# kevinh-e/BetaOne

Measured on AMD Instinct MI355X. Metric: mcts_nodes_per_sec, higher is better.
Workload: dtype f32 (3 x f16 split, f32 accumulate)

## Files before the change

betaone_amd/csrc/bo_engine.cpp:

```cpp
#include "../../include/betaone_engine.h"
#include "../../include/betaone_lab.h"

#include "bo_tree.h"
#include "bo_fastw.h"
#include "bo_info.h"
#include "bo_select_wide.h"
#include "bo_replay.h"
#include "bo_train.h"
#include "bo_metrics.h"
#include "bo_pgn.h"
#include "bo_san.h"
#include "bo_analyse.h"
#include "bo_reanalyse.h"
#include "bo_perft.h"
#include "bo_mate.h"
#include "bo_anchor.h"
#include "bo_book.h"
#include "bo_merge.h"
#include "bo_tb.h"
#include "bo_nn_fused.h"
#include "bo_conv.h"
#include "bo_tower.h"
#include "bo_tower_wg.h"
#include "bo_tower_h.h"
// ... 202 lines not shown
    e->fast = fast;
    double per_sim = 1.0;
    for (int k = 1; k <= cfg->mcts_batch_size; k++) {
        const double r = (double)(int)(cfg->widen_coeff * sqrt((double)k)) / (double)k;
        if (r > per_sim) per_sim = r;
    }
    c.NCAP = fast ? 2 : (int)ceil(c.S * per_sim) + 2 * root_m + 4;
    c.nstride = c.NCAP;
    c.PLY_CAP = cfg->max_plies; c.TRK_CAP = cfg->max_plies;
    c.UL_MAX = fast ? 1 : c.B; c.CH_MAX = ch_max < 1 ? 1 : ch_max;
    c.cpuct = (float)cfg->cpuct;
    c.keep = (float)(1.0 - cfg->dirichlet_epsilon);
    c.eps = cfg->dirichlet_epsilon;
    c.use_noise = cfg->dirichlet_alpha > 0 ? 1 : 0;
    c.root_m = root_m;
    c.profile = 0;
    { const char *v = getenv("BETAONE_BURST_TWO_PATHS"); c.burst_two = (v && v[0] == '0') ? 0 : 1; }
    c.root_q = 0;
    const size_t G = (size_t)c.G, N = G * (size_t)c.NCAP;
    Eng &d = e->d;
    int rc = 0;
    float *sq = nullptr, *rcp = nullptr; int *wl = nullptr;
    rc |= e->alloc(&sq, (size_t)c.S + 2); rc |= e->alloc(&wl, (size_t)c.B + 1); rc |= e->alloc(&rcp, (size_t)c.S + 3);
    int **iscal[] = {&d.sims_done, &d.n_nodes, &d.rows, &d.n_runs, &d.n_ul, &d.req_nlegal, &d.status,
                     &d.trk_n, &d.n_hist, &d.ctx_mode, &d.root_nch, &d.stat_evals,
                     &d.stat_flushes, &d.stat_term_sims, &d.stat_levels, &d.stat_children_scanned, &e->d_go, &e->d_action};
    for (int **p : iscal) rc |= e->alloc(p, G);
    const size_t res_ints = G * (4 + 2 * (size_t)BO_RES_CAP) + 4, info_ints = G * 18;
    rc |= e->alloc(&e->d_res_blk, res_ints); rc |= e->alloc(&e->d_info_blk, info_ints);
    if (!rc) {
        d.res_n = e->d_res_blk; d.res_best_idx = e->d_res_blk + G; d.res_best_mv = e->d_res_blk + 2 * G; d.res_total = e->d_res_blk + 3 * G;
        d.res_idx = e->d_res_blk + 4 * G; d.res_val = reinterpret_cast<float *>(e->d_res_blk + 4 * G + G * BO_RES_CAP);
        d.res_watch = e->d_res_blk + G * (4 + 2 * (size_t)BO_RES_CAP); d.watch = nullptr; d.watch_n = 1;
        d.phase = e->d_info_blk; d.req_node = e->d_info_blk + G; d.root_nlegal = e->d_info_blk + 2 * G; d.root_term = e->d_info_blk + 3 * G;
        d.ply = e->d_info_blk + 4 * G;
        e->d_turn_action = e->d_info_blk + 5 * G; e->d_turn_state = e->d_info_blk + 6 * G; e->d_turn_cres = e->d_info_blk + 7 * G;
        e->d_turn_rv = reinterpret_cast<float *>(e->d_info_blk + 15 * G); e->d_turn_resigned = e->d_info_blk + 16 * G;
        e->d_turn_rnext = e->d_info_blk + 17 * G;
        rt_memset(e->d_res_blk, 0, res_ints * 4, nullptr); rt_memset(e->d_info_blk, 0, info_ints * 4, nullptr);
    }
    rc |= rt_host_alloc((void **)&e->h_res, res_ints * 4); rc |= rt_host_alloc((void **)&e->h_info, info_ints * 4);
    rc |= rt_host_alloc((void **)&e->h_noise, G * BO_MAX_MOVES * sizeof(double)); rc |= rt_host_alloc((void **)&e->h_go, G * 4);
    rc |= rt_host_alloc((void **)&e->h_action, 2 * G * 4);
    rc |= rt_host_alloc((void **)&e->h_turn_u, G * sizeof(double)); rc |= rt_host_alloc((void **)&e->h_turn_flags, G * 4);
    rc |= e->alloc(&e->d_turn_pw, (size_t)cfg->num_simulations + 1);
    { const char *v = getenv("BETAONE_TURN_COPIES"); e->ship = !(v && v[0] == '1'); }
// ... 35 lines not shown
        rc |= e->alloc(&st, (size_t)BO_FW_SQRT_TAB); rc |= e->alloc(&rt, (size_t)BO_FW_RCP_TAB);
        if (!rc) {
            std::vector<float> hs2(BO_FW_SQRT_TAB), hr2(BO_FW_RCP_TAB, 0.0f);
            for (int n = 0; n < BO_FW_SQRT_TAB; n++) hs2[n] = (float)sqrt((double)n);
            for (int k = 1; k < BO_FW_RCP_TAB; k++) hr2[k] = (float)(1.0 / (double)k);
            rt_h2d(st, hs2.data(), hs2.size() * sizeof(float), nullptr); rt_h2d(rt, hr2.data(), hr2.size() * sizeof(float), nullptr);
            rt_sync(nullptr);
            f.sqrt_tab = st; f.rcp_tab = rt;
            rt_memset(f.ctl, 0, G * (size_t)f.CS * 4, nullptr);
            rt_memset(f.played_now, 0, G * 4, nullptr);
            rt_memset(f.row_val, 0, G * L * 4, nullptr);
            d.played_now = f.played_now;
        }
    }
    if (rc) { bo_engine_destroy(e); return fail(BO_E_HIP, "device allocation failed"); }
    std::vector<float> hs((size_t)c.S + 2);
    for (int n = 0; n < c.S + 2; n++) hs[n] = (float)sqrt((double)n + 1e-8);
    std::vector<int> hw((size_t)c.B + 1);
    for (int k = 0; k <= c.B; k++) hw[k] = (int)(cfg->widen_coeff * sqrt((double)k));
    std::vector<float> hr((size_t)c.S + 3, 0.0f);
    for (int n = 1; n < c.S + 3; n++) hr[n] = (float)(1.0 / (double)n);
    rt_h2d(rcp, hr.data(), hr.size() * sizeof(float), nullptr);
    d.rcp_lut = rcp;
    rt_h2d(sq, hs.data(), hs.size() * sizeof(float), nullptr);
    rt_h2d(wl, hw.data(), hw.size() * sizeof(int), nullptr);
    d.sqrt_lut = sq; d.widen_lut = wl;
    for (int **p : iscal) rt_memset(*p, 0, G * sizeof(int), nullptr);
    rt_memset(d.noise, 0, G * BO_MAX_MOVES * sizeof(double), nullptr);
    rt_sync(nullptr);
    e->h_i32.resize(G);
    e->rng.resize(G);
    for (size_t g = 0; g < G; g++) hr_seed(&e->rng[g], (uint32_t)g);
    memset(e->h_noise, 0, G * BO_MAX_MOVES * sizeof(double));
    e->h_nl.resize(G); e->h_term.resize(G);
    *out = e;
    return BO_OK;
}

extern "C" void bo_engine_destroy(bo_engine *e) {
    if (!e) return;
    rt_set_device(e->device);
    for (void *p : e->allocs) rt_free(p);
    rt_host_free(e->h_res); rt_host_free(e->h_info); rt_host_free(e->h_noise); rt_host_free(e->h_go); rt_host_free(e->h_action);
    rt_host_free(e->h_turn_u); rt_host_free(e->h_turn_flags);
    if (e->ev_turn_made) rt_event_destroy(e->ev_turn);
    for (int i = 0; i < 2; i++) if (e->ev_action_made[i]) rt_event_destroy(e->ev_action[i]);
// ... 191 lines not shown
static int step_launch(bo_engine *e, const float *policy_dev, const float *value_dev, int policy_kind, float *nn_in_dev, void *stream, const StepTail &vt) {
    e->prefetch_valid = false;
    if (e->fast) {
        const int rows = e->d.c.G * e->f.L;
        if (policy_kind != BO_POLICY_NONE) RT(RT_LAUNCH(bo_k_fw_apply, rows, stream, e->d, e->f, policy_dev, value_dev, policy_kind));
#if !defined(BO_WAVE_EMU)
        if (e->sel_profile) {
            if (!e->sel_ev0) { RT((int)hipEventCreate(&e->sel_ev0)); RT((int)hipEventCreate(&e->sel_ev1)); }
            if (e->sel_pending) {
                float ms = 0.0f;
                RT((int)hipEventSynchronize(e->sel_ev1));
                RT((int)hipEventElapsedTime(&ms, e->sel_ev0, e->sel_ev1));
                e->sel_ms += ms; e->sel_launches++; e->sel_pending = 0;
            }
            RT((int)hipEventRecord(e->sel_ev0, (hipStream_t)stream));
        }
#endif
        RT(launch_fw_select(e, policy_kind != BO_POLICY_NONE ? e->f.row_val : value_dev, policy_kind, stream));
#if !defined(BO_WAVE_EMU)
        if (e->sel_profile) { RT((int)hipEventRecord(e->sel_ev1, (hipStream_t)stream)); e->sel_pending = 1; }
#endif
        RT(RT_LAUNCH(bo_k_fw_leaf, rows, stream, e->d, e->f, nn_in_dev));
    } else {
        if (e->d.tb_n > 0 && (e->d.tb_flags & TBF_SEARCH)) RT(RT_LAUNCH(bo_k_step_tb, e->d.c.G, stream, e->d, policy_dev, value_dev, policy_kind, nn_in_dev, vt));
        else RT(RT_LAUNCH(bo_k_step, e->d.c.G, stream, e->d, policy_dev, value_dev, policy_kind, nn_in_dev, vt));
    }
    return BO_OK;
}
extern "C" int bo_step(bo_engine *e, const float *policy_dev, const float *value_dev, int policy_kind, float *nn_in_dev,
                       void *stream) {
    if (!e || !nn_in_dev) return fail(BO_E_ARG, "null argument");
    if (policy_kind != BO_POLICY_NONE && (!policy_dev || !value_dev)) return fail(BO_E_ARG, "policy/value required");
    return step_launch(e, policy_dev, value_dev, policy_kind, nn_in_dev, stream, StepTail{nullptr, nullptr, nullptr, nullptr, 0});
}
extern "C" int bo_step_heads(bo_engine *e, const float *logits_dev, const float *vpart_dev, const float *b1_dev, const float *w2_dev,
                             const float *b2_dev, int rows, float *nn_in_dev, void *stream) {
    if (!e || !nn_in_dev || !logits_dev || !vpart_dev || !b1_dev || !w2_dev || !b2_dev) return fail(BO_E_ARG, "null argument");
    if (e->fast) return fail(BO_E_CONFIG, "bo_step_heads: the reference-semantics search only (fast mode evaluates rows, not games)");
    if (rows < e->d.c.G) return fail(BO_E_ARG, "bo_step_heads: the partial sums must hold a row per game (rows >= G)");
    return step_launch(e, logits_dev, nullptr, BO_POLICY_LOGITS, nn_in_dev, stream, StepTail{vpart_dev, b1_dev, w2_dev, b2_dev, rows});
}

extern "C" int bo_search_poll(bo_engine *e, int32_t *n_running, int32_t *n_requested, int32_t *requested_mask, void *stream) {
    if (!e) return fail(BO_E_ARG, "null engine");
    const size_t G = (size_t)e->d.c.G;
    RT(rt_d2h(e->h_info, e->d_info_blk, 2 * G * 4, stream));
    const int *ph = e->h_info, *rq = e->h_info + G;
    RT(rt_sync(stream));
// ... 1558 lines not shown
        const size_t pitch = (size_t)e->f.CS * 4;
        if (term_sims) RT(rt_d2h_2d(term_sims, 4, e->f.ctl + FWC_TERM, pitch, 4, G, stream));
        if (levels) RT(rt_d2h_2d(levels, 4, e->f.ctl + FWC_LEVELS, pitch, 4, G, stream));
        if (children_scanned) RT(rt_d2h_2d(children_scanned, 4, e->f.ctl + FWC_KIDS, pitch, 4, G, stream));
    } else {
        if (term_sims) RT(rt_d2h(term_sims, e->d.stat_term_sims, G * 4, stream));
        if (levels) RT(rt_d2h(levels, e->d.stat_levels, G * 4, stream));
        if (children_scanned) RT(rt_d2h(children_scanned, e->d.stat_children_scanned, G * 4, stream));
    }
    RT(rt_sync(stream));
    return BO_OK;
}

extern "C" int bo_debug_profile(bo_engine *e, int enable, uint64_t *cycles_out, void *stream) {
    if (!e) return fail(BO_E_ARG, "null engine");
    const size_t G = (size_t)e->d.c.G;
    if (cycles_out) {
        RT(rt_d2h(cycles_out, e->d.prof, G * BO_PROF_SLOTS * sizeof(uint64_t), stream));
        RT(rt_sync(stream));
    }
    if (enable >= 0) {
        if (enable && !e->d.c.profile) RT(rt_memset(e->d.prof, 0, G * BO_PROF_SLOTS * sizeof(uint64_t), stream));
        e->d.c.profile = enable;
    }
    return BO_OK;
}

extern "C" int bo_movegen_batch(bo_engine *e, int n, const bo_position *pos, int32_t *moves_out, int32_t *n_out,
                                int32_t *check_out, void *stream) {
    if (!e || n < 1 || !pos || !moves_out || !n_out) return fail(BO_E_ARG, "bad arguments");
    std::vector<DPos> hp((size_t)n);
    for (int i = 0; i < n; i++) hp[i] = from_abi(pos[i]);
    void *dp = nullptr, *dm = nullptr, *dn = nullptr, *dc = nullptr;
    int rc = rt_malloc(&dp, hp.size() * sizeof(DPos)) | rt_malloc(&dm, (size_t)n * BO_MAX_MOVES * sizeof(bo_mv)) |
             rt_malloc(&dn, (size_t)n * 4) | rt_malloc(&dc, (size_t)n * 4);
    std::vector<bo_mv> hm((size_t)n * BO_MAX_MOVES);
    std::vector<int> hc((size_t)n);
    if (!rc) rc = rt_h2d(dp, hp.data(), hp.size() * sizeof(DPos), stream);
    if (!rc) rc = RT_LAUNCH(bo_k_movegen, n, stream, (const DPos *)dp, (bo_mv *)dm, (int *)dn, (int *)dc);
    if (!rc) rc = rt_d2h(hm.data(), dm, hm.size() * sizeof(bo_mv), stream) | rt_d2h(n_out, dn, (size_t)n * 4, stream) |
                  rt_d2h(hc.data(), dc, (size_t)n * 4, stream);
    int rc2 = rt_sync(stream);
    rt_free(dp); rt_free(dm); rt_free(dn); rt_free(dc);
    if (rc || rc2) return fail(BO_E_HIP, std::string("bo_movegen_batch: ") + rt_errstr(rc ? rc : rc2));
    for (size_t i = 0; i < hm.size(); i++) moves_out[i] = hm[i];
    if (check_out) for (int i = 0; i < n; i++) check_out[i] = hc[i];
// ... 1752 lines not shown
```

betaone_amd/csrc/bo_tree.h:

```cpp
#pragma once
#include "bo_chess.h"
#include "bo_tb_probe.h"
#include <math.h>

#define BO_CH_CAP 32
#define BO_PATH_CAP 1024
#define BO_RES_CAP 256
#define BO_PLANES 120
#ifndef BO_PROF_SLOTS
#define BO_PROF_SLOTS 16
#endif
#define BO_ROW (BO_PLANES * 64)

enum { PH_IDLE = 0, PH_RUN = 1, PH_DONE = 2 };
enum { ST_OK = 0, ST_NODE_OVERFLOW = 1, ST_DEPTH_OVERFLOW = 2, ST_NAN_SCORE = 4, ST_PLY_OVERFLOW = 8,
       ST_ILLEGAL_ACTION = 16, ST_UL_OVERFLOW = 32, ST_TRK_OVERFLOW = 64 };
enum { POLICY_NONE = 0, POLICY_LOGITS = 1, POLICY_PROBS = 2 };

struct EngCfg {
    int G, S, B;
    int NCAP, PLY_CAP, TRK_CAP;
    int nstride;
    int UL_MAX, CH_MAX;
    float cpuct, keep;
    double eps;
    int use_noise;
    int root_m;
    int profile;
    int burst_two;
    int root_q;
};

struct Eng {
    EngCfg c;
    const float *sqrt_lut;
    const float *rcp_lut;
    const int *widen_lut;
    int *phase, *sims_done, *n_nodes, *rows, *n_runs, *n_ul, *req_node, *req_nlegal, *status;
    int *ply, *trk_n, *n_hist, *ctx_mode, *root_nlegal, *root_term, *root_nch;
    int *stat_evals, *stat_flushes, *stat_term_sims, *stat_levels, *stat_children_scanned;
    DPos *gpos, *trk, *hist;
    int *trk_cnt;
    int *n_visits, *parent, *first_child, *n_children;
    float *q, *prior;
    bo_mv *move;
    signed char *term;
    short *eval_slot;
    DPos *npos;
    int *run_leaf, *run_cnt;
    int *ul_node, *ul_nlegal;
    float *ul_value;
    bo_mv *ul_move;
    float *ul_prior;
    bo_mv *req_moves, *root_moves;
    int *root_child_rank;
    double *noise;
    bo_mv *played;
    int *res_n, *res_idx, *res_best_idx, *res_best_mv, *res_total;
    float *res_val;
    int watch_n;
// ... 2 lines not shown
    int *resign_cnt;
    unsigned long long *prof;
    const TbTable *tb_tabs;
    int tb_n;
    int tb_flags;
    int *tb_stat;
};
enum { TBF_SEARCH = 1, TBF_ADJUDICATE = 2 };
enum { TERM_TB_WIN = 3, TERM_TB_LOSS = 4, TERM_TB_DRAW = 5 };

#define NOFF(e, g) ((size_t)(g) * (size_t)(e).c.nstride)

BO_DEV float bo_expf(float x) {
#if defined(BO_WAVE_EMU)
    return expf(x);
#else
    return __expf(x);
#endif
}
struct bo_f4 { float x, y, z, w; };
BO_DEV float bo_exp_row(float x) { return expf(x); }
#if defined(BO_WAVE_EMU)
#define BO_UNROLL
#else
#define BO_UNROLL _Pragma("unroll")
#endif
constexpr int BO_ROW_N4 = BO_NUM_ACTIONS / 4, BO_ROW_IT = (BO_ROW_N4 + 63) / 64;
BO_DEV float bo_wave_sum_desc_f(float v) {
    for (int m = 32; m >= 1; m >>= 1) v = v + bo_shfl_xor_f(v, m);
    return v;
}
BO_DEV void row_load_max_sum(const float *row, bo_f4 (&v)[BO_ROW_IT], float *mx_out, float *sum_out) {
    const bo_f4 *r4 = reinterpret_cast<const bo_f4 *>(row);
    const int lane = bo_lane();
    const float ninf = -__builtin_inff();
    BO_UNROLL
    for (int i = 0; i < BO_ROW_IT; i++) {
        const int k = lane + 64 * i;
        v[i] = k < BO_ROW_N4 ? r4[k] : bo_f4{ninf, ninf, ninf, ninf};
    }
    float mx = ninf;
    BO_UNROLL
    for (int i = 0; i < BO_ROW_IT; i++) {
        const float a = v[i].x > v[i].y ? v[i].x : v[i].y, b = v[i].z > v[i].w ? v[i].z : v[i].w;
        const float c = a > b ? a : b;
        mx = c > mx ? c : mx;
    }
    mx = bo_wave_max_f(mx);
// ... 416 lines not shown
            BO_BURST_STEP(0) BO_BURST_STEP(1) BO_BURST_STEP(2) BO_BURST_STEP(3)
#undef BO_BURST_STEP
            int bterm = (j == (bi & 15)) ? cterm : -2;
            { int o = BO_ROW_XCHG(bterm, 0); bterm = o > bterm ? o : bterm; }
            { int o = BO_ROW_XCHG(bterm, 1); bterm = o > bterm ? o : bterm; }
            { int o = BO_ROW_XCHG(bterm, 2); bterm = o > bterm ? o : bterm; }
            { int o = BO_ROW_XCHG(bterm, 3); bterm = o > bterm ? o : bterm; }
            const int src = 16 * (d - 1);
            const int nb = bo_readlane(bi, src), nt = bo_readlane(bterm, src);
            if (!(nt > 0)) break;
            if (last_l) my_chosen = nb;
            v_cur = nt == 1 ? 1.0f : 0.0f;
        }
    }
#undef BO_SQ
#undef BO_RC
    if (have) { e.n_visits[no + my_fc + j] = cn; e.q[no + my_fc + j] = cq; }
    if (two && b_have) { e.n_visits[no + b_fc + j] = b_cn; e.q[no + b_fc + j] = b_cq; }
    if (lane == 0) { e.n_visits[no] = nv[0]; if (root_q) e.q[no] = rq; }
    bo_sync();
    return done;
}

BO_DEV void backup_run(const Eng &e, int g, int leaf, float v, int cnt, int *scratch, int *flags, const int *known = nullptr,
                       int known_depth = -1) {
    const size_t no = NOFF(e, g);
    int d = 0;
    if (known_depth >= 0) {
        d = known_depth + 1;
    } else {
        for (int x = leaf; x >= 0 && d < BO_PATH_CAP; x = e.parent[no + x]) {
            if (bo_lane() == 0) scratch[d] = x;
            d++;
        }
        bo_sync();
    }
    for (int i = bo_lane(); i < d; i += 64) {
        const int nd = known_depth >= 0 ? known[known_depth - i] : scratch[i];
        const float val = (i & 1) ? -v : v;
        int n = e.n_visits[no + nd];
        float qv = e.q[no + nd];
        for (int c = 0; c < cnt; c++) {
            n += 1;
            const float dd = val - qv;
            const float ee = dd / (float)n;
            qv = qv + ee;
        }
        e.n_visits[no + nd] = n;
        e.q[no + nd] = qv;
    }
    bo_sync();
}

BO_DEV void init_node(const Eng &e, size_t no, int idx, int par, float prior, bo_mv m, const DPos &P) {
    e.n_visits[no + idx] = 0;
    e.q[no + idx] = 0.0f;
    e.prior[no + idx] = prior;
    e.parent[no + idx] = par;
    e.first_child[no + idx] = 0;
    e.n_children[no + idx] = 0;
    e.move[no + idx] = m;
    e.term[no + idx] = -1;
    e.eval_slot[no + idx] = -1;
    e.npos[no + idx] = P;
}

BO_DEV void flush_pending(const Eng &e, int g, int n_runs, int n_ul, int *n_nodes_io, int *path, int *flags, int cur_leaf = -1,
                          const int *cur_path = nullptr, int cur_depth = -1) {
    const size_t no = NOFF(e, g);
    const int lane = bo_lane();
    const int *rl = e.run_leaf + (size_t)g * e.c.B, *rc = e.run_cnt + (size_t)g * e.c.B;
    int n_nodes = *n_nodes_io;
// ... 158 lines not shown
        for (int ks = 0; ks < 16; ks++) r.part[w][ks] = t.vpart[((size_t)ks * t.rows + g) * 256 + lane + 64 * w];
        r.b1[w] = t.b1[lane + 64 * w];
        r.w2[w] = t.w2[lane + 64 * w];
    }
    r.b2 = t.b2[0];
}
BO_DEV float tail_value(const TailRegs &r) {
    float s[4];
    BO_UNROLL
    for (int w = 0; w < 4; w++) {
        float h = 0.0f;
        BO_UNROLL
        for (int ks = 0; ks < 16; ks++) h += r.part[w][ks];
        h += r.b1[w];
        s[w] = (h > 0.0f ? h : 0.0f) * r.w2[w];
    }
    for (int m = 32; m >= 1; m >>= 1) {
        BO_UNROLL
        for (int w = 0; w < 4; w++) s[w] = s[w] + bo_shfl_xor_f(s[w], m);
    }
    return tanhf(((s[0] + s[1]) + (s[2] + s[3])) + r.b2);
}

BO_DEV void apply_leaf(const Eng &e, int g, int leaf, const float *row, int kind, const float *value_of, const StepTail &vt, StepShared &sh,
                       int *n_ul_io, int *flags) {
    const size_t no = NOFF(e, g);
    const int lane = bo_lane();
    const int n = e.req_nlegal[g];
    const bo_mv *mv = e.req_moves + (size_t)g * BO_MAX_MOVES;
    int slot = *n_ul_io;
    if (slot >= e.c.UL_MAX) { *flags |= ST_UL_OVERFLOW; slot = e.c.UL_MAX - 1; }
    const size_t uo = (size_t)g * e.c.UL_MAX + slot;
    float value;
    bool bad = false;
    if (kind == POLICY_PROBS) {
        value = value_of[g];
        for (int j = lane; j < n; j += 64) sh.pv[j] = finite_or_zero(row[move_to_index(mv[j])], &bad);
    } else {
        float mx, sum;
        if (vt.vpart) {
            TailRegs tr;
            tail_load(vt, g, tr);
            row_max_sum(row, &mx, &sum);
            value = tail_value(tr);
        } else {
            value = value_of[g];
            row_max_sum(row, &mx, &sum);
        }
        for (int j = lane; j < n; j += 64) sh.pv[j] = finite_or_zero(bo_exp_row(row[move_to_index(mv[j])] - mx) / sum, &bad);
    }
    bo_sync();
    value = finite_or_zero(value, &bad);
    if (bo_ballot(bad) != 0) *flags |= ST_NAN_SCORE;
    const int M = n < e.c.CH_MAX ? n : e.c.CH_MAX;
    for (int j = lane; j < n; j += 64) {
        int r = stable_rank(sh.pv, n, j);
        if (r < M) { e.ul_move[uo * BO_CH_CAP + r] = mv[j]; e.ul_prior[uo * BO_CH_CAP + r] = sh.pv[j]; }
    }
    if (lane == 0) {
        e.ul_node[uo] = leaf;
        e.ul_nlegal[uo] = n;
        e.ul_value[uo] = value;
        e.eval_slot[no + leaf] = (short)slot;
    }
    *n_ul_io = slot + 1;
    bo_sync();
}


BO_DEV float tb_leaf_value(int t, int kc) {
    const float m = 1.0f - (float)kc * (1.0f / 1024.0f);
    return t == TERM_TB_LOSS ? m : t == TERM_TB_WIN ? -m : 0.0f;
}
template <bool TB>
BO_DEV int step_body(const Eng &e, int g, const float *policy, const float *value, int kind, float *nn_in, StepShared &sh, const StepTail &vt) {
    const int lane = bo_lane();
    const size_t no = NOFF(e, g);
    int flags = 0;
    int sims = e.sims_done[g], rows = e.rows[g], n_runs = e.n_runs[g], n_ul = e.n_ul[g], n_nodes = e.n_nodes[g];
    int req = e.req_node[g];
    int *rl = e.run_leaf + (size_t)g * e.c.B, *rc = e.run_cnt + (size_t)g * e.c.B;
    float *row = nn_in + (size_t)g * BO_ROW;

    const bool prof = e.c.profile != 0;
    unsigned long long pc[8] = {0, 0, 0, 0, 0, 0, 0, 0};
    int n_iter = 0, n_first = 0, n_burst = 0, n_burst_sims = 0, n_general = 0, n_swaps = 0;
    unsigned long long tk = prof ? bo_clock() : 0ull;
    const unsigned long long t_start = tk;
#define BO_PROF(slot)                                                    \
    if (prof) { const unsigned long long _n = bo_clock(); pc[slot] += _n - tk; tk = _n; }
    if (req >= 0 && kind == POLICY_NONE) return n_nodes;
    const float *lut = e.sqrt_lut;
    if (req >= 0) {
        if (req == 0) apply_root(e, g, policy + (size_t)g * BO_NUM_ACTIONS, kind, sh, &n_nodes, &flags);
        else apply_leaf(e, g, req, policy + (size_t)g * BO_NUM_ACTIONS, kind, value, vt, sh, &n_ul, &flags);
        req = -1;
    }
    BO_PROF(0)
    int phase = PH_RUN;
    bool burst_tables_staged = false;
    int term_budget = e.c.B;
    int b_depth = 0;
    float b_tv = 0.0f;
    int path_leaf = -1, path_depth = -1;
    for (;;) {
        if (sims >= e.c.S) {
            if (rows > 0) { flush_pending(e, g, n_runs, n_ul, &n_nodes, sh.path2, &flags, path_leaf, sh.path, path_depth); rows = n_runs = n_ul = 0; }
            BO_PROF(5)
            phase = PH_DONE;
            break;
        }
        int depth;
        const int leaf = select_leaf(e, g, &flags, sh.path, &depth, lut);
        path_leaf = leaf; path_depth = depth;
        n_iter++;
        BO_PROF(1)
        int t = e.term[no + leaf];
        int tb_k = 0;
        if (TB && t >= TERM_TB_WIN) tb_k = (int)e.eval_slot[no + leaf];
        if (t < 0) {
            n_first++;
            const DPos P = e.npos[no + leaf];
            bool chk;
            const int n = bo_movegen(P, sh.moves, &chk);
            t = terminal_eval(e, g, sh.path, depth, P, sh.moves, n, chk, sh.moves2, sh.chain);
            if constexpr (TB) {
                const bool gate = t == 0 && leaf != 0 && (e.tb_flags & TBF_SEARCH) && bo_popc64(P.bb[BB_WHITE] | P.bb[BB_BLACK]) <= TB_MAX_MEN &&
                                  !(P.flags & F_CASTLE_MASK);
                if (bo_uniform(gate ? 1 : 0)) {
                    const uint32_t code = tb_lookup(e.tb_tabs, e.tb_n, P.bb, pos_turn(P));
                    const int k = (int)code - 2;
                    if (code == 1u) t = TERM_TB_DRAW;
                    else if (code >= 2u && code != TB_NO_TABLE && P.halfmove + k <= 100) t = (k & 1) ? TERM_TB_WIN : TERM_TB_LOSS;
                    if (t != 0) {
                        tb_k = t == TERM_TB_DRAW ? 0 : k < 512 ? k : 512;
                        if (lane == 0) { e.eval_slot[no + leaf] = (short)tb_k; e.tb_stat[3 * g] += 1; }
// ... 20 lines not shown
            if (small) {
                const bool small_b = b_depth > 0 && e.c.burst_two != 0;
                applied = terminal_burst<TB>(e, g, sh.path, depth, tv, may, sh.probs, &burst_tables_staged, sh.bpath, tb_leaf ? -1 : small_b ? b_depth : 0, b_tv,
                                             &n_swaps);
                n_burst++; n_burst_sims += applied;
                bo_sync();
                if (lane <= depth) sh.bpath[lane] = sh.path[lane];
                b_depth = tb_leaf ? 0 : depth; b_tv = tv;
                bo_sync();
            }
            else { backup_run(e, g, leaf, tv, 1, sh.path2, &flags, sh.path, depth); n_general++; }
            BO_PROF(7)
            sims += applied;
            term_budget -= applied;
            if (lane == 0) e.stat_term_sims[g] += applied;
            if (tb_leaf && lane == 0) e.tb_stat[3 * g + 1] += applied;
            BO_PROF(3)
            if (term_budget <= 0 && sims < e.c.S) break;
            continue;
        }
        if (e.eval_slot[no + leaf] < 0) {
            encode_leaf(e, g, row, e.npos[no + leaf]);
            req = leaf;
            if (lane == 0) e.stat_evals[g] += 1;
            BO_PROF(4)
            break;
        }
        int cnt = e.c.B - rows;
        if (cnt > e.c.S - sims) cnt = e.c.S - sims;
        if (lane == 0) { rl[n_runs] = leaf; rc[n_runs] = cnt; }
        n_runs++;
        rows += cnt;
        sims += cnt;
        bo_sync();
        if (rows >= e.c.B) { flush_pending(e, g, n_runs, n_ul, &n_nodes, sh.path2, &flags, path_leaf, sh.path, path_depth); rows = n_runs = n_ul = 0; }
        BO_PROF(5)
    }
#undef BO_PROF
    if (prof && lane == 0) {
        const unsigned long long total = bo_clock() - t_start;
        if (e.c.profile == 1 || total > (unsigned long long)e.c.profile) {
            unsigned long long *pp = e.prof + (size_t)g * BO_PROF_SLOTS;
            pp[10] += (unsigned long long)n_burst; pp[11] += (unsigned long long)n_burst_sims; pp[12] += (unsigned long long)n_general;
            pp[13] += pc[6]; pp[14] += pc[7]; pp[15] += (unsigned long long)n_swaps;
            for (int i = 0; i < 6; i++) pp[i] += pc[i];
            pp[6] += total;
            pp[7] += 1;
            pp[8] += (unsigned long long)n_iter;
            pp[9] += (unsigned long long)n_first;
        }
    }
    if (lane == 0) {
        e.sims_done[g] = sims; e.rows[g] = rows; e.n_runs[g] = n_runs; e.n_ul[g] = n_ul; e.n_nodes[g] = n_nodes;
        e.req_node[g] = req; e.phase[g] = phase;
        if (flags) e.status[g] |= flags;
    }
    return n_nodes;
}
BO_KERNEL void bo_k_step(Eng e, const float *policy, const float *value, int kind, float *nn_in, StepTail vt) {
    BO_SHARED StepShared sh;
    const int g = bo_block();
    if (e.phase[g] != PH_RUN) return;
    step_body<false>(e, g, policy, value, kind, nn_in, sh, vt);
}
BO_KERNEL void bo_k_step_tb(Eng e, const float *policy, const float *value, int kind, float *nn_in, StepTail vt) {
    BO_SHARED StepShared sh;
    const int g = bo_block();
    if (e.phase[g] != PH_RUN) return;
    step_body<true>(e, g, policy, value, kind, nn_in, sh, vt);
}

BO_DEV int root_prepare(const Eng &e, int g, StepShared &sh) {
    const size_t no = NOFF(e, g);
    const int lane = bo_lane();
    const int ply = e.ply[g];
    const DPos P = e.gpos[(size_t)g * e.c.PLY_CAP + ply];
    if (lane == 0) {
        init_node(e, no, 0, -1, 1.0f, 0, P);
        e.n_nodes[g] = 1; e.sims_done[g] = 0; e.rows[g] = 0; e.n_runs[g] = 0; e.n_ul[g] = 0;
        e.req_node[g] = -1; e.phase[g] = PH_IDLE; e.root_nch[g] = 0;
        if (e.ctx_mode[g] == 0) {
            int nh = ply < 7 ? ply : 7;
            e.n_hist[g] = nh;
            for (int i = 0; i < nh; i++) e.hist[(size_t)g * 7 + i] = e.gpos[(size_t)g * e.c.PLY_CAP + ply - nh + i];
        }
    }
    bo_sync();
    bool chk;
    const int n = bo_movegen(P, sh.moves, &chk);
    if (lane == 0) sh.path[0] = 0;
    bo_sync();
    int t = terminal_eval(e, g, sh.path, 0, P, sh.moves, n, chk, sh.moves2, sh.chain);
    int adj = 0;
// ... 354 lines not shown
```

betaone_amd/engine.py:

```python
from __future__ import annotations

import ctypes as C
import os
from typing import Dict, List, Optional, Sequence, Tuple

import numpy as np
import torch

NUM_ACTIONS = 4672
INPUT_CHANNELS = 120
ROW_FLOATS = 120 * 64
MAX_LEGAL = 256
RES_CAP = 256
POLICY_NONE, POLICY_LOGITS, POLICY_PROBS = 0, 1, 2

STATUS_BITS = {1: "node overflow", 2: "depth overflow", 4: "NaN or infinite evaluation (prior or value)", 8: "ply overflow",
               16: "illegal action", 32: "leaf cache overflow", 64: "tracker overflow", 128: "position range outside the array",
               256: "pi wider than the record's rows"}
ST_PLY_OVERFLOW, ST_ILLEGAL_ACTION = 8, 16
ST_PI_OVERFLOW = 256
ST_NODE_OVERFLOW = 1
ST_DEPTH_OVERFLOW = 2
ST_NAN_SCORE = 4

# ... 186 lines not shown
    "bo_pgn_movetext": (C.c_int, [C.c_int32, C.c_void_p, C.c_void_p, C.c_int32, C.c_int32, C.c_void_p, C.c_char_p, C.c_char_p, C.c_int64,
                                  C.POINTER(C.c_int64)]),
    "bo_perft": (C.c_int, [C.c_int, C.c_int32, C.POINTER(C.c_char_p), C.c_int32, C.c_int64, C.c_uint32, C.c_void_p, C.c_void_p, C.c_void_p,
                           C.POINTER(C.c_int64), C.c_void_p]),
    "bo_tb_create": (C.c_int, [C.c_int, C.c_char_p, C.POINTER(C.c_void_p), C.c_int32, C.POINTER(C.c_void_p)]),
    "bo_tb_build": (C.c_int, [C.c_void_p, C.c_int32, _I32P, C.c_void_p]),
    "bo_tb_verify": (C.c_int, [C.c_void_p, C.POINTER(C.c_uint64), C.c_void_p]),
    "bo_tb_stats": (C.c_int, [C.c_void_p, C.c_void_p]),
    "bo_tb_download": (C.c_int, [C.c_void_p, C.c_void_p, C.c_int64]),
    "bo_tb_upload": (C.c_int, [C.c_void_p, C.c_void_p, C.c_int64, C.c_int32]),
    "bo_tb_probe": (C.c_int, [C.POINTER(C.c_void_p), C.c_int32, C.c_void_p, C.c_int32, C.c_void_p, C.c_void_p, C.c_void_p]),
    "bo_engine_tablebases": (C.c_int, [C.c_void_p, C.POINTER(C.c_void_p), C.c_int32, C.c_int32]),
    "bo_engine_tb_stats": (C.c_int, [C.c_void_p, _I32P, _I32P, _I32P, C.c_void_p]),
    "bo_tb_destroy": (None, [C.c_void_p]),
    "bo_mate": (C.c_int, [C.c_int, C.c_int32, C.POINTER(C.c_char_p), C.c_void_p, C.c_int32, C.c_int64, C.c_uint64, C.c_uint32, C.c_void_p,
                          C.c_void_p, C.c_void_p, C.POINTER(C.c_int64), C.c_void_p]),
    "bo_anchor": (C.c_int, [C.c_int, C.c_int32, C.POINTER(C.c_char_p), C.c_void_p, C.c_int32, C.c_int64, C.c_uint32, C.c_void_p, C.c_void_p,
                            C.c_void_p, C.POINTER(C.c_int64), C.c_void_p]),
    "bo_anchor_eval": (C.c_int, [C.c_int, C.c_int32, C.c_void_p, C.c_void_p, C.c_void_p]),
}
_LAB_SYMBOLS = {
    "bo_debug_tree": (C.c_int, [C.c_void_p, C.c_int, C.POINTER(BoNode), C.c_int32, _I32P, C.c_void_p]),
    "bo_debug_search_state": (C.c_int, [C.c_void_p, _I32P, C.c_void_p]),
    "bo_debug_fast": (C.c_int, [C.c_void_p, C.c_int, _I32P, C.c_int32, _I32P, C.c_void_p]),
    "bo_event_pair_overhead": (C.c_int, [_F64P, C.c_int32, C.c_void_p]),
    "bo_nn_b1_profile": (C.c_int, [C.c_void_p, C.c_int, C.POINTER(C.c_uint64), C.c_int]),
    "bo_fast_stats": (C.c_int, [C.c_void_p, C.POINTER(C.c_uint64), C.POINTER(C.c_uint64), _I32P, C.c_int32, _F64P, C.POINTER(C.c_int64),
                               C.c_void_p]),
    "bo_debug_profile": (C.c_int, [C.c_void_p, C.c_int, C.POINTER(C.c_uint64), C.c_void_p]),
    "bo_debug_stamp": (C.c_int, [C.c_void_p, C.c_uint64, C.c_uint64, C.c_void_p]),
    "bo_nn_tower_forward_timed": (C.c_int, [C.c_void_p, C.c_void_p, C.c_void_p, C.c_void_p, C.c_void_p, C.c_int, C.c_void_p, C.c_void_p]),
    "bo_select_wide": (C.c_int, [C.c_void_p, C.c_void_p, C.c_void_p, C.c_void_p, C.c_int, C.c_int, C.c_float, C.c_int,
                                 C.c_void_p, C.c_void_p, C.c_void_p]),
}

HIP_LIB_PATH = os.path.join(os.path.dirname(os.path.abspath(__file__)), "csrc", "libbetaone_hip.so")


def bind(cdll: C.CDLL) -> C.CDLL:
    for name, (res, args) in list(_SYMBOLS.items()) + list(_LAB_SYMBOLS.items()):
        fn = getattr(cdll, name)
        fn.restype = res
        fn.argtypes = args
    return cdll


# ... 453 lines not shown
```

include/betaone_lab.h:

```cpp
#ifndef BETAONE_LAB_H
#define BETAONE_LAB_H

#include "betaone_engine.h"

#ifdef __cplusplus
extern "C" {
#endif

#define BO_PROF_SLOTS 16

typedef struct {
    int32_t parent, n_visits, first_child, n_children;
    float q_value, prior;
    int32_t move;
    int32_t terminal;
} bo_node;
int bo_debug_tree(bo_engine *e, int slot, bo_node *out, int32_t cap, int32_t *n_nodes, void *stream);
int bo_debug_search_state(bo_engine *e, int32_t *out, void *stream);

int bo_fast_stats(bo_engine *e, uint64_t *granules_read, uint64_t *path_nodes, int32_t *arena_granules, int32_t time_select, double *select_ms,
                  int64_t *select_launches, void *stream);

int bo_event_pair_overhead(double *ms_out, int32_t samples, void *stream);

int bo_debug_fast(bo_engine *e, int slot, int32_t *ctl_out, int32_t ctl_cap, int32_t *paths_out, void *stream);

int bo_debug_profile(bo_engine *e, int enable, uint64_t *cycles_out, void *stream);

int bo_select_wide(const void *blocks_dev, const int32_t *root_block_dev, const int32_t *root_n_dev,
                   const float *sqrt_lut_dev, int n_trees, int max_depth, float cpuct, int grid_blocks,
                   int32_t *out_leaf_dev, int32_t *out_levels_dev, void *stream);

int bo_nn_tower_forward_timed(bo_tower *tower, const float *x_dev, float *y_dev, void *head_a_dev, void *head_b_dev, int batch,
                              void *timing_dev, void *stream);

int bo_debug_stamp(void *ring_dev, uint64_t tag, uint64_t capacity, void *stream);

int bo_nn_b1_profile(bo_b1 *tower, int enable, uint64_t *out, int cap);

#ifdef __cplusplus
}
#endif
#endif
```

Measured before the change: 79.80 million.

## Use reciprocal table in backup, resume kept path, specialize step kernels

Backup replaces the per-visit float division with a multiply by a double-precision reciprocal looked up from a table. Loads are prefetched eight ahead, and the code falls back to exact division when a difference is tiny or a count is out of range. The step kernel saves the selected path for each game when it requests an evaluation, so the next step can resume at that leaf without re-running selection. Step kernels are also templated on tail and profiling, removing dead profiling and tail branches from the default kernel. These changes add a per-game path buffer and extra device memory, and the reciprocal multiply can round slightly differently from true division.

Result: no change. 81.56 million (median of 2 runs) (+2.2%).

```diff
diff --git a/betaone_amd/csrc/bo_engine.cpp b/betaone_amd/csrc/bo_engine.cpp
--- a/betaone_amd/csrc/bo_engine.cpp
+++ b/betaone_amd/csrc/bo_engine.cpp
@@ -248,6 +248,9 @@
     int rc = 0;
     float *sq = nullptr, *rcp = nullptr; int *wl = nullptr;
     rc |= e->alloc(&sq, (size_t)c.S + 2); rc |= e->alloc(&wl, (size_t)c.B + 1); rc |= e->alloc(&rcp, (size_t)c.S + 3);
+    double *rcp64 = nullptr;
+    rc |= e->alloc(&rcp64, (size_t)c.S + 3 + BO_BQ_AHEAD);
+    rc |= e->alloc(&d.path_row, fast ? 1 : G * BO_PATH_CAP); rc |= e->alloc(&d.path_depth, G);
     int **iscal[] = {&d.sims_done, &d.n_nodes, &d.rows, &d.n_runs, &d.n_ul, &d.req_nlegal, &d.status,
                      &d.trk_n, &d.n_hist, &d.ctx_mode, &d.root_nch, &d.stat_evals,
                      &d.stat_flushes, &d.stat_term_sims, &d.stat_levels, &d.stat_children_scanned, &e->d_go, &e->d_action};
@@ -329,6 +332,11 @@
     for (int n = 1; n < c.S + 3; n++) hr[n] = (float)(1.0 / (double)n);
     rt_h2d(rcp, hr.data(), hr.size() * sizeof(float), nullptr);
     d.rcp_lut = rcp;
+    std::vector<double> hr64((size_t)c.S + 3 + BO_BQ_AHEAD, 0.0);
+    for (int n = 1; n < (int)hr64.size(); n++) hr64[n] = bo_rcp64(n);
+    rt_h2d(rcp64, hr64.data(), hr64.size() * sizeof(double), nullptr);
+    d.rcp64_lut = rcp64;
+    rt_memset(d.path_depth, 0xFF, G * sizeof(int), nullptr);
     rt_h2d(sq, hs.data(), hs.size() * sizeof(float), nullptr);
     rt_h2d(wl, hw.data(), hw.size() * sizeof(int), nullptr);
     d.sqrt_lut = sq; d.widen_lut = wl;
@@ -566,8 +574,18 @@
 #endif
         RT(RT_LAUNCH(bo_k_fw_leaf, rows, stream, e->d, e->f, nn_in_dev));
     } else {
-        if (e->d.tb_n > 0 && (e->d.tb_flags & TBF_SEARCH)) RT(RT_LAUNCH(bo_k_step_tb, e->d.c.G, stream, e->d, policy_dev, value_dev, policy_kind, nn_in_dev, vt));
-        else RT(RT_LAUNCH(bo_k_step, e->d.c.G, stream, e->d, policy_dev, value_dev, policy_kind, nn_in_dev, vt));
+        const bool tb = e->d.tb_n > 0 && (e->d.tb_flags & TBF_SEARCH);
+        const int G = e->d.c.G;
+        if (e->d.c.profile) {
+            if (tb) RT(RT_LAUNCH(bo_k_step_tb_prof, G, stream, e->d, policy_dev, value_dev, policy_kind, nn_in_dev, vt));
+            else RT(RT_LAUNCH(bo_k_step_prof, G, stream, e->d, policy_dev, value_dev, policy_kind, nn_in_dev, vt));
+        } else if (vt.vpart) {
+            if (tb) RT(RT_LAUNCH(bo_k_step_tb_tail, G, stream, e->d, policy_dev, value_dev, policy_kind, nn_in_dev, vt));
+            else RT(RT_LAUNCH(bo_k_step_tail, G, stream, e->d, policy_dev, value_dev, policy_kind, nn_in_dev, vt));
+        } else {
+            if (tb) RT(RT_LAUNCH(bo_k_step_tb, G, stream, e->d, policy_dev, value_dev, policy_kind, nn_in_dev));
+            else RT(RT_LAUNCH(bo_k_step, G, stream, e->d, policy_dev, value_dev, policy_kind, nn_in_dev));
+        }
     }
     return BO_OK;
 }
@@ -2172,6 +2190,17 @@
     if (enable >= 0) {
         if (enable && !e->d.c.profile) RT(rt_memset(e->d.prof, 0, G * BO_PROF_SLOTS * sizeof(uint64_t), stream));
         e->d.c.profile = enable;
+    }
+    return BO_OK;
+}
+
+extern "C" int bo_debug_backup_quotient(const float *dd, const int32_t *n, float *out, uint8_t *took_division, int64_t count) {
+    if (!dd || !n || !out || count < 0) return fail(BO_E_ARG, "bad arguments");
+    for (int64_t i = 0; i < count; i++) {
+        if (n[i] < 1) return fail(BO_E_ARG, "bo_debug_backup_quotient: n must be >= 1");
+        const bool table = bo_backup_quot_ok(dd[i]);
+        out[i] = table ? bo_backup_quot(dd[i], bo_rcp64(n[i])) : dd[i] / (float)n[i];
+        if (took_division) took_division[i] = table ? 0 : 1;
     }
     return BO_OK;
 }
diff --git a/betaone_amd/csrc/bo_tree.h b/betaone_amd/csrc/bo_tree.h
--- a/betaone_amd/csrc/bo_tree.h
+++ b/betaone_amd/csrc/bo_tree.h
@@ -36,6 +36,9 @@
     const float *sqrt_lut;
     const float *rcp_lut;
     const int *widen_lut;
+    const double *rcp64_lut;
+    int *path_row;
+    int *path_depth;
     int *phase, *sims_done, *n_nodes, *rows, *n_runs, *n_ul, *req_node, *req_nlegal, *status;
     int *ply, *trk_n, *n_hist, *ctx_mode, *root_nlegal, *root_term, *root_nch;
     int *stat_evals, *stat_flushes, *stat_term_sims, *stat_levels, *stat_children_scanned;
@@ -84,8 +87,10 @@
 BO_DEV float bo_exp_row(float x) { return expf(x); }
 #if defined(BO_WAVE_EMU)
 #define BO_UNROLL
+#define BO_UNROLL_2
 #else
 #define BO_UNROLL _Pragma("unroll")
+#define BO_UNROLL_2 _Pragma("unroll 2")
 #endif
 constexpr int BO_ROW_N4 = BO_NUM_ACTIONS / 4, BO_ROW_IT = (BO_ROW_N4 + 63) / 64;
 BO_DEV float bo_wave_sum_desc_f(float v) {
@@ -548,32 +553,87 @@
     return done;
 }
 
+#if defined(BO_WAVE_EMU)
+#define BO_HOST_DEV static inline
+#else
+#define BO_HOST_DEV __host__ __device__ __forceinline__
+#endif
+BO_HOST_DEV double bo_rcp64(int n) { return 1.0 / (double)n; }
+BO_HOST_DEV float bo_backup_quot(float dd, double r) { return (float)((double)dd * r); }
+BO_HOST_DEV bool bo_backup_quot_ok(float dd) { return __builtin_fabsf(dd) >= 0x1p-100f || dd == 0.0f; }
+#define BO_BQ_AHEAD 8
 BO_DEV void backup_run(const Eng &e, int g, int leaf, float v, int cnt, int *scratch, int *flags, const int *known = nullptr,
                        int known_depth = -1) {
     const size_t no = NOFF(e, g);
+    const int lane = bo_lane();
     int d = 0;
     if (known_depth >= 0) {
         d = known_depth + 1;
     } else {
         for (int x = leaf; x >= 0 && d < BO_PATH_CAP; x = e.parent[no + x]) {
-            if (bo_lane() == 0) scratch[d] = x;
+            if (lane == 0) scratch[d] = x;
             d++;
         }
         bo_sync();
     }
-    for (int i = bo_lane(); i < d; i += 64) {
-        const int nd = known_depth >= 0 ? known[known_depth - i] : scratch[i];
+    const bool v_ok = __builtin_fabsf(v) < __builtin_inff() && e.rcp64_lut != nullptr;
+    for (int base = 0; base < d; base += 64) {
+        const int i = base + lane;
+        const bool act = i < d;
+        int nd = 0, n = 0;
+        float qv = 0.0f;
+        if (act) {
+            nd = known_depth >= 0 ? known[known_depth - i] : scratch[i];
+            n = e.n_visits[no + nd];
+            qv = e.q[no + nd];
+        }
         const float val = (i & 1) ? -v : v;
-        int n = e.n_visits[no + nd];
-        float qv = e.q[no + nd];
-        for (int c = 0; c < cnt; c++) {
-            n += 1;
-            const float dd = val - qv;
-            const float ee = dd / (float)n;
-            qv = qv + ee;
-        }
-        e.n_visits[no + nd] = n;
-        e.q[no + nd] = qv;
+        const int n0 = n;
+        const float q0 = qv;
+        bool redo = !(v_ok && bo_ballot(act && !(n >= 0 && n <= e.c.S + 2 - cnt)) == 0);
+        if (!redo && act) {
+            const double *R = e.rcp64_lut + n + 1;
+            int tiny = 0;
+            double r[BO_BQ_AHEAD], rn[BO_BQ_AHEAD];
+#define BO_BQ_STEP(rv)                                         \
+            {                                                  \
+                const float dd = val - qv;                     \
+                if (!bo_backup_quot_ok(dd)) tiny = 1;          \
+                qv = qv + bo_backup_quot(dd, (rv));            \
+            }
+            BO_UNROLL
+            for (int k = 0; k < BO_BQ_AHEAD; k++) r[k] = R[k];
+            int c = 0;
+            BO_UNROLL_2
+            for (; c + BO_BQ_AHEAD <= cnt; c += BO_BQ_AHEAD) {
+                BO_UNROLL
+                for (int k = 0; k < BO_BQ_AHEAD; k++) rn[k] = R[c + BO_BQ_AHEAD + k];
+                BO_UNROLL
+                for (int k = 0; k < BO_BQ_AHEAD; k++) BO_BQ_STEP(r[k])
+                BO_UNROLL
+                for (int k = 0; k < BO_BQ_AHEAD; k++) r[k] = rn[k];
+            }
+            BO_UNROLL
+            for (int k = 0; k < BO_BQ_AHEAD; k++)
+                if (c + k < cnt) BO_BQ_STEP(r[k])
+#undef BO_BQ_STEP
+            n += cnt;
+            redo = tiny != 0;
+        }
+        if (redo && act) {
+            n = n0;
+            qv = q0;
+            for (int c = 0; c < cnt; c++) {
+                n += 1;
+                const float dd = val - qv;
+                const float ee = dd / (float)n;
+                qv = qv + ee;
+            }
+        }
+        if (act) {
+            e.n_visits[no + nd] = n;
+            e.q[no + nd] = qv;
+        }
     }
     bo_sync();
 }
@@ -778,6 +838,7 @@
     return tanhf(((s[0] + s[1]) + (s[2] + s[3])) + r.b2);
 }
 
+template <bool TAIL>
 BO_DEV void apply_leaf(const Eng &e, int g, int leaf, const float *row, int kind, const float *value_of, const StepTail &vt, StepShared &sh,
                        int *n_ul_io, int *flags) {
     const size_t no = NOFF(e, g);
@@ -794,7 +855,7 @@
         for (int j = lane; j < n; j += 64) sh.pv[j] = finite_or_zero(row[move_to_index(mv[j])], &bad);
     } else {
         float mx, sum;
-        if (vt.vpart) {
+        if (TAIL && vt.vpart) {
             TailRegs tr;
             tail_load(vt, g, tr);
             row_max_sum(row, &mx, &sum);
@@ -828,28 +889,40 @@
     const float m = 1.0f - (float)kc * (1.0f / 1024.0f);
     return t == TERM_TB_LOSS ? m : t == TERM_TB_WIN ? -m : 0.0f;
 }
-template <bool TB>
+template <bool TB, bool TAIL, bool PROF>
 BO_DEV int step_body(const Eng &e, int g, const float *policy, const float *value, int kind, float *nn_in, StepShared &sh, const StepTail &vt) {
     const int lane = bo_lane();
     const size_t no = NOFF(e, g);
     int flags = 0;
     int sims = e.sims_done[g], rows = e.rows[g], n_runs = e.n_runs[g], n_ul = e.n_ul[g], n_nodes = e.n_nodes[g];
     int req = e.req_node[g];
+    const int *kept = e.path_row + (size_t)g * BO_PATH_CAP;
+    int kept_depth = e.path_depth[g];
+    const int kept_mine = kept[lane];
     int *rl = e.run_leaf + (size_t)g * e.c.B, *rc = e.run_cnt + (size_t)g * e.c.B;
     float *row = nn_in + (size_t)g * BO_ROW;
 
-    const bool prof = e.c.profile != 0;
+    const bool prof = PROF && e.c.profile != 0;
     unsigned long long pc[8] = {0, 0, 0, 0, 0, 0, 0, 0};
     int n_iter = 0, n_first = 0, n_burst = 0, n_burst_sims = 0, n_general = 0, n_swaps = 0;
     unsigned long long tk = prof ? bo_clock() : 0ull;
     const unsigned long long t_start = tk;
 #define BO_PROF(slot)                                                    \
-    if (prof) { const unsigned long long _n = bo_clock(); pc[slot] += _n - tk; tk = _n; }
+    if (PROF && prof) { const unsigned long long _n = bo_clock(); pc[slot] += _n - tk; tk = _n; }
     if (req >= 0 && kind == POLICY_NONE) return n_nodes;
     const float *lut = e.sqrt_lut;
+    int resume_leaf = -1;
     if (req >= 0) {
         if (req == 0) apply_root(e, g, policy + (size_t)g * BO_NUM_ACTIONS, kind, sh, &n_nodes, &flags);
-        else apply_leaf(e, g, req, policy + (size_t)g * BO_NUM_ACTIONS, kind, value, vt, sh, &n_ul, &flags);
+        else {
+            apply_leaf<TAIL>(e, g, req, policy + (size_t)g * BO_NUM_ACTIONS, kind, value, vt, sh, &n_ul, &flags);
+            if (kept_depth >= 1 && kept_depth < BO_PATH_CAP) {
+                if (lane <= kept_depth) sh.path[lane] = kept_mine;
+                for (int i = lane + 64; i <= kept_depth; i += 64) sh.path[i] = kept[i];
+                bo_sync();
+                if (sh.path[0] == 0 && sh.path[kept_depth] == req) resume_leaf = req;
+            }
+        }
         req = -1;
     }
     BO_PROF(0)
@@ -859,6 +932,7 @@
     int b_depth = 0;
     float b_tv = 0.0f;
     int path_leaf = -1, path_depth = -1;
+    int out_depth = -1;
     for (;;) {
         if (sims >= e.c.S) {
             if (rows > 0) { flush_pending(e, g, n_runs, n_ul, &n_nodes, sh.path2, &flags, path_leaf, sh.path, path_depth); rows = n_runs = n_ul = 0; }
@@ -866,8 +940,9 @@
             phase = PH_DONE;
             break;
         }
-        int depth;
-        const int leaf = select_leaf(e, g, &flags, sh.path, &depth, lut);
+        int depth, leaf;
+        if (resume_leaf > 0) { leaf = resume_leaf; depth = kept_depth; resume_leaf = -1; }
+        else leaf = select_leaf(e, g, &flags, sh.path, &depth, lut);
         path_leaf = leaf; path_depth = depth;
         n_iter++;
         BO_PROF(1)
@@ -934,6 +1009,10 @@
         if (e.eval_slot[no + leaf] < 0) {
             encode_leaf(e, g, row, e.npos[no + leaf]);
             req = leaf;
+            if (leaf > 0) {
+                for (int i = lane; i <= depth; i += 64) e.path_row[(size_t)g * BO_PATH_CAP + i] = sh.path[i];
+                out_depth = depth;
+            }
             if (lane == 0) e.stat_evals[g] += 1;
             BO_PROF(4)
             break;
@@ -949,7 +1028,7 @@
         BO_PROF(5)
     }
 #undef BO_PROF
-    if (prof && lane == 0) {
+    if (PROF && prof && lane == 0) {
         const unsigned long long total = bo_clock() - t_start;
         if (e.c.profile == 1 || total > (unsigned long long)e.c.profile) {
             unsigned long long *pp = e.prof + (size_t)g * BO_PROF_SLOTS;
@@ -964,23 +1043,35 @@
     }
     if (lane == 0) {
         e.sims_done[g] = sims; e.rows[g] = rows; e.n_runs[g] = n_runs; e.n_ul[g] = n_ul; e.n_nodes[g] = n_nodes;
-        e.req_node[g] = req; e.phase[g] = phase;
+        e.req_node[g] = req; e.phase[g] = phase; e.path_depth[g] = out_depth;
         if (flags) e.status[g] |= flags;
     }
     return n_nodes;
 }
-BO_KERNEL void bo_k_step(Eng e, const float *policy, const float *value, int kind, float *nn_in, StepTail vt) {
+#define BO_STEP_KERNEL(name, TB, TAIL, PROF)                                                                          \
+    BO_KERNEL void name(Eng e, const float *policy, const float *value, int kind, float *nn_in, StepTail vt) {        \
+        BO_SHARED StepShared sh;                                                                                      \
+        const int g = bo_block();                                                                                     \
+        if (e.phase[g] != PH_RUN) return;                                                                             \
+        step_body<TB, TAIL, PROF>(e, g, policy, value, kind, nn_in, sh, vt);                                          \
+    }
+BO_KERNEL void bo_k_step(Eng e, const float *policy, const float *value, int kind, float *nn_in) {
     BO_SHARED StepShared sh;
     const int g = bo_block();
     if (e.phase[g] != PH_RUN) return;
-    step_body<false>(e, g, policy, value, kind, nn_in, sh, vt);
-}
-BO_KERNEL void bo_k_step_tb(Eng e, const float *policy, const float *value, int kind, float *nn_in, StepTail vt) {
+    step_body<false, false, false>(e, g, policy, value, kind, nn_in, sh, StepTail{nullptr, nullptr, nullptr, nullptr, 0});
+}
+BO_KERNEL void bo_k_step_tb(Eng e, const float *policy, const float *value, int kind, float *nn_in) {
     BO_SHARED StepShared sh;
     const int g = bo_block();
     if (e.phase[g] != PH_RUN) return;
-    step_body<true>(e, g, policy, value, kind, nn_in, sh, vt);
-}
+    step_body<true, false, false>(e, g, policy, value, kind, nn_in, sh, StepTail{nullptr, nullptr, nullptr, nullptr, 0});
+}
+BO_STEP_KERNEL(bo_k_step_tail, false, true, false)
+BO_STEP_KERNEL(bo_k_step_tb_tail, true, true, false)
+BO_STEP_KERNEL(bo_k_step_prof, false, true, true)
+BO_STEP_KERNEL(bo_k_step_tb_prof, true, true, true)
+#undef BO_STEP_KERNEL
 
 BO_DEV int root_prepare(const Eng &e, int g, StepShared &sh) {
     const size_t no = NOFF(e, g);
diff --git a/betaone_amd/engine.py b/betaone_amd/engine.py
--- a/betaone_amd/engine.py
+++ b/betaone_amd/engine.py
@@ -232,6 +232,7 @@
 _LAB_SYMBOLS = {
     "bo_debug_tree": (C.c_int, [C.c_void_p, C.c_int, C.POINTER(BoNode), C.c_int32, _I32P, C.c_void_p]),
     "bo_debug_search_state": (C.c_int, [C.c_void_p, _I32P, C.c_void_p]),
+    "bo_debug_backup_quotient": (C.c_int, [C.c_void_p, C.c_void_p, C.c_void_p, C.c_void_p, C.c_int64]),
     "bo_debug_fast": (C.c_int, [C.c_void_p, C.c_int, _I32P, C.c_int32, _I32P, C.c_void_p]),
     "bo_event_pair_overhead": (C.c_int, [_F64P, C.c_int32, C.c_void_p]),
     "bo_nn_b1_profile": (C.c_int, [C.c_void_p, C.c_int, C.POINTER(C.c_uint64), C.c_int]),
diff --git a/include/betaone_lab.h b/include/betaone_lab.h
--- a/include/betaone_lab.h
+++ b/include/betaone_lab.h
@@ -27,6 +27,8 @@
 
 int bo_debug_profile(bo_engine *e, int enable, uint64_t *cycles_out, void *stream);
 
+int bo_debug_backup_quotient(const float *dd, const int32_t *n, float *out, uint8_t *took_division, int64_t count);
+
 int bo_select_wide(const void *blocks_dev, const int32_t *root_block_dev, const int32_t *root_n_dev,
                    const float *sqrt_lut_dev, int n_trees, int max_depth, float cpuct, int grid_blocks,
                    int32_t *out_leaf_dev, int32_t *out_levels_dev, void *stream);
```
